# hanmekim/SceneLib2

Hardware: NVIDIA H100
Metric: EKF-SLAM frames/sec @320x240 N=100 feats (higher is better)
Workload: dtype f64 (EKF, scores) + u8/int32 (correlation sums)

## Files before the change

scenelib2_b200/csrc/update.cu:

```cuda
#include <type_traits>

#include "sl2_context.cuh"
#include "sl2_ptx.cuh"

using namespace sl2;

namespace {

constexpr int UPD_THREADS = 256;
constexpr int UPD_NB = 16;
constexpr int UPD_WS = 20;
constexpr int UPD_DS = 20;
constexpr int UPD_MS = 20;
constexpr int UPD_YS = 68;
constexpr int SOLVE_MAX_WARPS = 8;

__host__ __device__ inline int upd_keven(int kmax) { return (kmax + 1) & ~1; }
__host__ __device__ inline int upd_panw(int kmax) {
  return ((2 * upd_keven(kmax) + 15) & ~15) + 2;
}
__host__ __device__ inline size_t upd_pan_doubles(int kmax) { return (size_t)UPD_NB * upd_panw(kmax); }

__device__ __forceinline__ void dmma884(double &c0, double &c1, double a, double b) {
  asm("mma.sync.aligned.m8n8k4.row.col.f64.f64.f64.f64 {%0,%1}, {%2}, {%3}, {%0,%1};"
      : "+d"(c0), "+d"(c1)
      : "d"(a), "d"(b));
}
__device__ __forceinline__ void dmma1684(double (&c)[4], const double (&a)[2], double b) {
  asm("mma.sync.aligned.m16n8k4.row.col.f64.f64.f64.f64 {%0,%1,%2,%3}, {%4,%5}, {%6}, {%0,%1,%2,%3};"
      : "+d"(c[0]), "+d"(c[1]), "+d"(c[2]), "+d"(c[3])
      : "d"(a[0]), "d"(a[1]), "d"(b));
}
__device__ __forceinline__ void dmma1688(double (&c)[4], const double (&a)[4], const double (&b)[2]) {
  asm("mma.sync.aligned.m16n8k8.row.col.f64.f64.f64.f64 {%0,%1,%2,%3}, {%4,%5,%6,%7}, {%8,%9}, {%0,%1,%2,%3};"
      : "+d"(c[0]), "+d"(c[1]), "+d"(c[2]), "+d"(c[3])
      : "d"(a[0]), "d"(a[1]), "d"(a[2]), "d"(a[3]), "d"(b[0]), "d"(b[1]));
}
__device__ __forceinline__ void cp_async_commit() { asm volatile("cp.async.commit_group;" ::: "memory"); }
template <int N>
__device__ __forceinline__ void cp_async_wait() {
  asm volatile("cp.async.wait_group %0;" ::"n"(N) : "memory");
}
__device__ __forceinline__ void bulk_g2s(void *smem_dst, const void *gsrc, uint32_t bytes, uint32_t bar) {
  asm volatile("cp.async.bulk.shared::cluster.global.mbarrier::complete_tx::bytes [%0], [%1], %2, [%3];" ::"r"(
                   smem_u32(smem_dst)),
               "l"(gsrc), "r"(bytes), "r"(bar)
               : "memory");
}

__device__ __forceinline__ double pivot_rsqrt(double dv) {
  double y;
  asm("rsqrt.approx.ftz.f64 %0, %1;" : "=d"(y) : "d"(dv));
#pragma unroll
  for (int it = 0; it < 2; ++it) {
    const double e = fma(-(dv * y), y, 1.0);
    y = fma(0.5 * y, e, y);
  }
  return y;
}

__device__ __forceinline__ void chol8_inv(double *dg, double *Wm, int o, int lane) {
  const int j = lane & 7;
  double a[8], w[8];
#pragma unroll
  for (int i = 0; i < 8; ++i) {
    a[i] = (i <= j) ? dg[(o + i) * UPD_DS + o + j] : 0.0;
    w[i] = (i == j) ? 1.0 : 0.0;
  }
#pragma unroll
  for (int r = 0; r < 8; ++r) {
    const double dv = __shfl_sync(0xffffffffu, a[r], r);
    const double iu = pivot_rsqrt(dv);
    const double urj = a[r] * iu;
    a[r] = urj;
    w[r] *= iu;
#pragma unroll
    for (int i = r + 1; i < 8; ++i) {
      const double uri = __shfl_sync(0xffffffffu, urj, i);
      a[i] -= uri * urj;
      w[i] -= uri * w[r];
    }
  }
  __syncwarp();
  if (lane < 8) {
#pragma unroll
    for (int i = 0; i < 8; ++i) {
      if (i <= j) dg[(o + i) * UPD_DS + o + j] = a[i];
      Wm[(o + i) * UPD_WS + o + j] = w[i];
    }
  }
}

constexpr int HP_THREADS = 320;
constexpr int HP_ROWS = 16;
constexpr int HP_HRS = 18;
struct HpSmem {
  double *Hrow;
  double *Rv;
  double *nu;
  double *hprow;
  int *mfeat;
  int *wcount;
  double *park;
};
struct HpLayout {
  size_t Hrow, Rv, nu, hprow, mfeat, wcount, park, bytes;
};
__host__ __device__ inline HpLayout hp_layout(int kmax, int ld, int kd_park) {
  const size_t K = upd_keven(kmax);
  HpLayout l;
  l.Hrow = 0;
  l.Rv = l.Hrow + 2 * K * HP_HRS * sizeof(double);
  l.nu = l.Rv + 3 * K * sizeof(double);
  l.hprow = l.nu + 2 * K * sizeof(double);
  l.mfeat = l.hprow + (size_t)HP_ROWS * ld * sizeof(double);
  l.wcount = l.mfeat + K * sizeof(int);
  l.park = l.wcount + 16 * sizeof(int);
  l.bytes = l.park + (size_t)kd_park * HP_THREADS * sizeof(double);
  return l;
}
__device__ __forceinline__ HpSmem hp_carve(uint8_t *base, int kmax, int ld) {
  const HpLayout l = hp_layout(kmax, ld, 0);
  HpSmem u;
  u.Hrow = reinterpret_cast<double *>(base + l.Hrow);
  u.Rv = reinterpret_cast<double *>(base + l.Rv);
  u.nu = reinterpret_cast<double *>(base + l.nu);
  u.hprow = reinterpret_cast<double *>(base + l.hprow);
  u.mfeat = reinterpret_cast<int *>(base + l.mfeat);
  u.wcount = reinterpret_cast<int *>(base + l.wcount);
  u.park = reinterpret_cast<double *>(base + l.park);
  return u;
}

__device__ __forceinline__ int hp_tables(const Sl2Dev &d, const HpSmem &sm, int s, int rows_per_block, int row_found,
                                         int staged_m,
                                         const int *st_feat, const double *st_Hxv, const double *st_Hy,
                                         const double *st_R, const double *st_nu, const Sl2Subpix &sp,
                                         const Sl2Iter &it) {
  const int tid = threadIdx.x;
  const size_t fb = (size_t)s * d.Nmax;
  const bool iter_rows = it.h && staged_m < 0 && row_found == 1;
  const bool iter_pass = iter_rows && it.pass >= 0;
  const bool skip = iter_pass && !(it.pass == 0 ? it.max_it[s] > 0 : it.active[s] != 0);
  const bool relin = iter_rows && it.pass != 0 && it.max_it[s] > 0 && it.iters[s] > 0;
  const double *const tab_h = relin ? it.h : d.h;
  const double *const tab_dxp = relin ? it.Hxp : d.dh_dxp;
  const double *const tab_dy = relin ? it.Hy : d.dh_dy;
  int K;
  if (staged_m >= 0) {
    K = staged_m / 2;
    for (int k = tid; k < K; k += HP_THREADS) sm.mfeat[k] = st_feat[k];
  } else {
    const int nsel = d.nsel[s];
    int feat = -1;
    if (!skip && tid < d.Nmax && tid < nsel) {
      const int i = d.job_feat[fb + tid];
      if (i >= 0 && d.found[fb + i] == row_found) feat = i;
    }
    K = block_gather(feat, sm.mfeat, sm.wcount, (SL2_MAX_MEASURED + 31) / 32);
  }
  const int m = 2 * K;
  if (blockIdx.x == 0 && tid == 0) {
    d.upd_m[s] = m;
    if (staged_m < 0 && row_found == 1) {
      if (!iter_pass) d.nmeas[s] = K;
    } else if (staged_m < 0 && K > 0) {
      d.nmeas[s] += K;
    }
// ... 427 lines not shown
          chol8_inv(dg, sm.Wm, 0, lane);
          __syncwarp();
          {
            double c0 = 0.0, c1 = 0.0;
#pragma unroll
            for (int ks = 0; ks < 2; ++ks)
              dmma884(c0, c1, sm.Wm[lr * UPD_WS + 4 * ks + lc], dg[(4 * ks + lc) * UPD_DS + 8 + lr]);
            __syncwarp();
            *reinterpret_cast<double2 *>(dg + lr * UPD_DS + 8 + 2 * lc) = make_double2(c0, c1);
          }
          __syncwarp();
          {
            double2 cv = *reinterpret_cast<const double2 *>(dg + (8 + lr) * UPD_DS + 8 + 2 * lc);
#pragma unroll
            for (int ks = 0; ks < 2; ++ks) {
              const double v = dg[(4 * ks + lc) * UPD_DS + 8 + lr];
              dmma884(cv.x, cv.y, -v, v);
            }
            *reinterpret_cast<double2 *>(dg + (8 + lr) * UPD_DS + 8 + 2 * lc) = cv;
          }
          __syncwarp();
          chol8_inv(dg, sm.Wm, 8, lane);
          __syncwarp();
          {
            double t0 = 0.0, t1 = 0.0;
#pragma unroll
            for (int ks = 0; ks < 2; ++ks)
              dmma884(t0, t1, dg[(4 * ks + lc) * UPD_DS + 8 + lr], sm.Wm[(4 * ks + lc) * UPD_WS + lr]);
            *reinterpret_cast<double2 *>(dg + (8 + lr) * UPD_DS + 2 * lc) = make_double2(t0, t1);
            __syncwarp();
            double w0 = 0.0, w1 = 0.0;
#pragma unroll
            for (int ks = 0; ks < 2; ++ks)
              dmma884(w0, w1, -sm.Wm[(8 + lr) * UPD_WS + 8 + 4 * ks + lc], dg[(8 + 4 * ks + lc) * UPD_DS + lr]);
            *reinterpret_cast<double2 *>(sm.Wm + (8 + lr) * UPD_WS + 2 * lc) = make_double2(w0, w1);
          }
          __syncwarp();
          if (nbp < UPD_NB)
            for (int e = lane; e < UPD_NB * UPD_NB; e += 32) {
              const int i = e >> 4, j = e & 15;
              if (i >= nbp || j >= nbp) sm.Wm[i * UPD_WS + j] = 0.0;
            }
        }
      } else if (it == 1) {
        if (nbn == 0) continue;
        double c[2][4];
#pragma unroll
        for (int q = 0; q < 2; ++q)
#pragma unroll
          for (int mt = 0; mt < 2; ++mt) {
            const int r = mt * 8 + lr, cc = 8 * q + 2 * lc;
            c[q][2 * mt] = (r < nbn && n0 + cc < width) ? G[(size_t)(n0 + r) * ldg + n0 + cc] : 0.0;
            c[q][2 * mt + 1] = (r < nbn && n0 + cc + 1 < width) ? G[(size_t)(n0 + r) * ldg + n0 + cc + 1] : 0.0;
          }
        double v[CH_D][2];
        const size_t kstride = (size_t)4 * ldg;
        const double *gpre = G + (size_t)lc * ldg + n0 + lr;
        double *mp = mnext + lc * UPD_MS + lr;
        const bool v0 = lr < nbn, v1 = 8 + lr < nbn;
        auto loadv = [&](double *dst) {
          const double x0 = gpre[0], x1 = gpre[8];
          dst[0] = v0 ? -x0 : 0.0;
          dst[1] = v1 ? -x1 : 0.0;
          gpre += kstride;
        };
        auto step = [&](const double *vu) {
          const double a[2] = {vu[0], vu[1]};
          mp[0] = a[0];
          mp[8] = a[1];
          mp += 4 * UPD_MS;
          dmma1684(c[0], a, -a[0]);
          dmma1684(c[1], a, -a[1]);
        };
#pragma unroll
        for (int u = 0; u < CH_D - 1; ++u)
          if (u < nk) loadv(v[u]);
        int kb = 0;
        for (; kb + CH_D <= nk; kb += CH_D) {
#pragma unroll
          for (int u = 0; u < CH_D; ++u) {
            if (kb + u + CH_D - 1 < nk) loadv(v[(u + CH_D - 1) % CH_D]);
            step(v[u]);
          }
        }
#pragma unroll
        for (int q = 0; q < 2; ++q)
#pragma unroll
          for (int mt = 0; mt < 2; ++mt)
            *reinterpret_cast<double2 *>(dnext + (mt * 8 + lr) * CH_DPS + 8 * q + 2 * lc) =
                make_double2(c[q][2 * mt], c[q][2 * mt + 1]);
      } else {
        const int bt = it - 2;
        if (gb == 4) chol_batch<4, 4>(G, ldg, mcur, sm.pan, PW, i0, nbp, nk, ngroups, width, 2 + bt * 4, lr, lc);
        else if (gb == 2) chol_batch<2, 8>(G, ldg, mcur, sm.pan, PW, i0, nbp, nk, ngroups, width, 2 + bt * 2, lr, lc);
        else chol_batch<1, 8>(G, ldg, mcur, sm.pan, PW, i0, nbp, nk, ngroups, width, 2 + bt, lr, lc);
      }
    }
    __syncthreads();
    const int ncol = width - i0;
    for (int e = tid; e < UPD_NB * UPD_NB; e += UPD_THREADS) {
      const int r = e / UPD_NB, cc = e - r * UPD_NB;
      if (r < nbp && cc < nbp && i0 + cc < width)
        G[(size_t)(i0 + r) * ldg + i0 + cc] = (cc >= r) ? sm.dg[r * UPD_DS + cc] : 0.0;
      Wp[(size_t)pidx * 256 + e] = sm.Wm[r * UPD_WS + cc];
      if (r >= nbp || UPD_NB + cc >= ncol) mnext[(i0 + r) * UPD_MS + cc] = 0.0;
    }
    if (tid == 0) s_next = 1;
    {
      double aw[4][2];
#pragma unroll
      for (int mt = 0; mt < 2; ++mt)
#pragma unroll
        for (int ks = 0; ks < 4; ++ks) aw[ks][mt] = sm.Wm[(mt * 8 + lr) * UPD_WS + 4 * ks + lc];
      constexpr int FG = 4;
      for (int gb = 2 + warp; gb * 8 < ncol; gb += FG * (UPD_THREADS / 32)) {
        double c[FG][4];
#pragma unroll
        for (int f = 0; f < FG; ++f) c[f][0] = c[f][1] = c[f][2] = c[f][3] = 0.0;
#pragma unroll
        for (int ks = 0; ks < 4; ++ks) {
          double bv[FG];
#pragma unroll
          for (int f = 0; f < FG; ++f) {
            const int cb = (gb + f * (UPD_THREADS / 32)) * 8 + lr;
            bv[f] = cb < ncol ? sm.pan[(size_t)(4 * ks + lc) * PW + cb] : 0.0;
          }
#pragma unroll
          for (int f = 0; f < FG; ++f) dmma1684(c[f], aw[ks], bv[f]);
        }
#pragma unroll
        for (int f = 0; f < FG; ++f) {
          const int gq = gb + f * (UPD_THREADS / 32);
          const int cc = gq * 8 + 2 * lc;
#pragma unroll
          for (int mt = 0; mt < 2; ++mt) {
            const int r = mt * 8 + lr;
            if (r < nbp && cc < ncol) {
              double *dst = G + (size_t)(i0 + r) * ldg + i0 + cc;
              if (cc + 1 < ncol) *reinterpret_cast<double2 *>(dst) = make_double2(c[f][2 * mt], c[f][2 * mt + 1]);
              else *dst = c[f][2 * mt];
              if (gq < 4) {
                mnext[(i0 + r) * UPD_MS + cc - UPD_NB] = -c[f][2 * mt];
                if (cc + 1 < ncol) mnext[(i0 + r) * UPD_MS + cc + 1 - UPD_NB] = -c[f][2 * mt + 1];
              }
            }
          }
        }
      }
    }
    __syncthreads();
  }
}

__device__ __forceinline__ double c_to_b(const double (&c)[2][2], int ks, int lane) {
  const int lr = lane >> 2, lc = lane & 3;
  const int src = ((4 * (ks & 1) + lc) << 2) | (lr >> 1);
  const double v0 = __shfl_sync(0xffffffffu, c[ks >> 1][0], src);
  const double v1 = __shfl_sync(0xffffffffu, c[ks >> 1][1], src);
  return (lr & 1) ? v1 : v0;
}

template <int NP> struct SolveLayout {
  static constexpr int SPLIT = NP > 13 ? 6 : NP;
  static constexpr int REUSE = NP > 13 ? 4 : NP;
  __host__ __device__ static constexpr int pw(int p) { return 16 * (NP - 1 - p) + 4; }
  __host__ __device__ static constexpr int off_lin(int p0, int p) {
    int o = 0;
    for (int q = p0; q < p; ++q) o += 16 * pw(q);
    return o;
  }
  __host__ __device__ static constexpr int off(int p) { return p < SPLIT ? off_lin(0, p) : off_lin(SPLIT, p); }
  static constexpr int PAN_DOUBLES = off_lin(0, SPLIT < NP - 1 ? SPLIT : NP - 1);
  static constexpr int SMEM_DOUBLES = PAN_DOUBLES + NP * 16 * UPD_WS + NP + (NP & 1) +
                                      2 * SOLVE_MAX_WARPS * 2 * 32 * 2 +
                                      SOLVE_MAX_WARPS * 128;
  static_assert(SPLIT == NP || off_lin(SPLIT, NP - 1) <= off_lin(0, REUSE), "second generation must fit");
};

template <int NP>
__global__ void __launch_bounds__(64 * SOLVE_MAX_WARPS, 1) upd_solve_kernel(const Sl2Dev d, int stream_lo) {
  using L = SolveLayout<NP>;
  extern __shared__ __align__(16) uint8_t smem_raw[];
  pdl_prologue();
  double *pan = reinterpret_cast<double *>(smem_raw);
  double *Wm = pan + L::PAN_DOUBLES;
  const uint32_t bars = smem_u32(Wm + NP * 16 * UPD_WS);
  double2 *xbuf = reinterpret_cast<double2 *>(Wm + NP * 16 * UPD_WS + NP + (NP & 1));
  double *ybuf = reinterpret_cast<double *>(xbuf + 2 * SOLVE_MAX_WARPS * 2 * 32);
  const int s = stream_lo + blockIdx.y;
  const int m = d.upd_m[s];
  if (m == 0) return;
  const int tid = threadIdx.x, nthr = blockDim.x;
  const int ngrp = nthr >> 6;
  const int warp = tid >> 5, lane = tid & 31, lr = lane >> 2, lc = lane & 3;
  const int g = warp % ngrp, rho = warp / ngrp;
  const int n = SL2_NXV + 3 * d.nfeat[s];
  const int ncols = n + 1;
  if (blockIdx.x * ngrp * 8 >= ncols) return;
  const int ldg = d.ldg;
  double *__restrict__ G = d.G + (size_t)s * d.mmax * ldg;
  const double *__restrict__ Wp = d.Wp + (size_t)s * SL2_MAX_PANELS * 256;
  const int m8 = (m + 7) & ~7;
  const bool full = L::SPLIT == NP && m8 >= 16 * NP - 8;
  const int zend = full ? 16 * NP : m8;

  if (tid == 0) {
    for (int p = 0; p < NP; ++p) mbar_init(bars + 8 * p, 1);
    fence_barrier_init();
    fence_proxy_async();
  }
  auto zero_pads = [&](int plo, int phi) {
    for (int e = tid; e < (phi - plo) * 16; e += nthr) {
      const int p = plo + (e >> 4), r = e & 15;
      const int cfirst = 16 * p + 16;
      if (16 * p < m)
        for (int c = max(m, cfirst); c < zend; ++c) pan[L::off(p) + r * L::pw(p) + (c - cfirst)] = 0.0;
    }
  };
  zero_pads(0, L::SPLIT);
  __syncthreads();
  auto request = [&](int p) {
    if (16 * p < m) {
      const int cfirst = 16 * p + 16;
      const int nrow = min(16, m - 16 * p);
      const uint32_t ubytes = m > cfirst ? (uint32_t)(m - cfirst) * 8u : 0u;
      const uint32_t bar = bars + 8 * p;
      if (lane == 0) mbar_expect_tx(bar, (uint32_t)nrow * ubytes + 16u * 128u);
      __syncwarp();
      if (lane < 16) {
        if (lane < nrow && ubytes)
          bulk_g2s(pan + L::off(p) + lane * L::pw(p), G + (size_t)(16 * p + lane) * ldg + cfirst, ubytes, bar);
      } else {
        bulk_g2s(Wm + ((size_t)p * 16 + (lane - 16)) * UPD_WS, Wp + (size_t)p * 256 + (lane - 16) * 16, 128u, bar);
      }
    }
  };
  if (warp == 0) {
#pragma unroll 1
    for (int p = 0; p < L::SPLIT; ++p) request(p);
  }

  int xpar = 0;
  auto solve_group = [&](auto full_c, const int grp) {
    constexpr bool FULL = decltype(full_c)::value;
    const int c0 = 8 * grp;
    const bool wact = c0 < ncols;
    const int cc = c0 + 2 * lc;
    const int cval = wact ? min(2, ncols - cc) : 0;
    double *gcol = G + m + cc;
    double acc[(NP + 1) & ~1][2];
    {
      const int ccn = cc + 8 * (int)(gridDim.x * ngrp);
      if (L::SPLIT >= NP && ccn < ncols) {
#pragma unroll
        for (int t = 0; t < NP; ++t) {
          const int row = 8 * (2 * t + rho) + lr;
          if (row < m) asm volatile("prefetch.global.L2 [%0];" ::"l"(G + m + ccn + (size_t)row * ldg));
        }
      }
    }
#pragma unroll
    for (int t = 0; t < ((NP + 1) & ~1); ++t) {
      const int row = 8 * (2 * t + rho) + lr;
      acc[t][0] = acc[t][1] = 0.0;
      if (row < m) {
        if (cval >= 2) {
          const double2 v = *reinterpret_cast<const double2 *>(gcol + (size_t)row * ldg);
          acc[t][0] = v.x;
          acc[t][1] = v.y;
        } else if (cval == 1) {
          acc[t][0] = gcol[(size_t)row * ldg];
        }
      }
    }

#pragma unroll
    for (int p = 0; p < NP; ++p) {
      if (FULL || 16 * p < m) {
        if (L::SPLIT < NP && p == L::REUSE) {
          __syncthreads();
          zero_pads(L::SPLIT, NP);
          __syncthreads();
          if (warp == 0) {
            fence_proxy_async();
#pragma unroll 1
            for (int q = L::SPLIT; q < NP; ++q) request(q);
          }
        }
        if (!wact) continue;
        xpar ^= 1;
        double2 *xb = xbuf + ((size_t)(xpar * ngrp + g) * 2) * 32;
        xb[rho * 32 + lane] = make_double2(acc[p][0], acc[p][1]);
        asm volatile("bar.sync %0, 64;" ::"r"(1 + g) : "memory");
        const double2 other = xb[(rho ^ 1) * 32 + lane];
        const double cp2[2][2] = {{rho ? other.x : acc[p][0], rho ? other.y : acc[p][1]},
                                  {rho ? acc[p][0] : other.x, rho ? acc[p][1] : other.y}};
        mbar_wait(bars + 8 * p, 0);
        const double *pb = pan + L::off(p);
        const int PW = L::pw(p);
        const double *wb = Wm + (size_t)p * 16 * UPD_WS;
        double cb[4];
#pragma unroll
        for (int ks = 0; ks < 4; ++ks) cb[ks] = c_to_b(cp2, ks, lane);
        double d0 = 0.0, d1 = 0.0;
#pragma unroll
        for (int ks = 0; ks < 4; ++ks) dmma884(d0, d1, wb[(8 * rho + lr) * UPD_WS + 4 * ks + lc], cb[ks]);
        {
          const int row = 16 * p + 8 * rho + lr;
          if (row < m) {
            if (cval >= 2) *reinterpret_cast<double2 *>(gcol + (size_t)row * ldg) = make_double2(d0, d1);
            else if (cval == 1) gcol[(size_t)row * ldg] = d0;
          }
        }
        if (p + 1 < NP) {
          double *yg = ybuf + (size_t)g * 128;
          *reinterpret_cast<double2 *>(yg + (8 * rho + lr) * 8 + 2 * lc) = make_double2(d0, d1);
          asm volatile("bar.sync %0, 64;" ::"r"(1 + g) : "memory");
          double yb[4];
#pragma unroll
          for (int ks = 0; ks < 4; ++ks) yb[ks] = -yg[(4 * ks + lc) * 8 + lr];
          const double *pbr = pb + 8 * rho + lr;
#pragma unroll
          for (int ks = 0; ks < 4; ++ks) {
#pragma unroll
            for (int t = (p + 1) & ~1; t < NP; t += 2) {
              const bool has[2] = {t > p && (FULL || 8 * (2 * t + rho) < m),
                                   t + 1 < NP && (FULL || 8 * (2 * t + 2 + rho) < m)};
              if (has[0] || has[1]) {
                double a[2];
#pragma unroll
                for (int h = 0; h < 2; ++h) a[h] = has[h] ? pbr[(4 * ks + lc) * PW + 16 * (t + h - p - 1)] : 0.0;
                double c[4] = {acc[t][0], acc[t][1], acc[t + 1][0], acc[t + 1][1]};
                dmma1684(c, a, yb[ks]);
                acc[t][0] = c[0];
                acc[t][1] = c[1];
                acc[t + 1][0] = c[2];
                acc[t + 1][1] = c[3];
              }
            }
          }
        }
      }
    }
  };
  for (int grp = blockIdx.x * ngrp + g; L::SPLIT < NP ? grp == (int)(blockIdx.x * ngrp + g) : 8 * grp < ncols;
       grp += gridDim.x * ngrp) {
    if (L::SPLIT == NP && full) solve_group(std::true_type{}, grp);
    else solve_group(std::false_type{}, grp);
  }
}

constexpr int SYRK_THREADS = 128;
template <int KC, int ST>
__global__ void __launch_bounds__(SYRK_THREADS, 3) upd_syrk_kernel(const Sl2Dev d, int stream_lo) {
  constexpr int STAGE = 2 * KC * UPD_YS;
  constexpr int NW = SYRK_THREADS / 32;
  extern __shared__ __align__(16) uint8_t smem_raw[];
  double *stage_buf = reinterpret_cast<double *>(smem_raw);
  pdl_prologue();
  const int s = stream_lo + blockIdx.y;
  const int m = d.upd_m[s];
  if (m == 0) return;
  const int n = SL2_NXV + 3 * d.nfeat[s];
  int tb = 0;
  const int t = blockIdx.x;
  while ((tb + 1) * (tb + 2) / 2 <= t) ++tb;
  const int ta = t - tb * (tb + 1) / 2;
  if (tb * 64 >= n + 1) return;
  const int tid = threadIdx.x, warp = tid >> 5, lane = tid & 31, lr = lane >> 2, lc = lane & 3;
  const int wa = (warp & 1) * 32, wb = (warp >> 1) * 32;
  const int ld = d.ld, ldg = d.ldg;
  double *__restrict__ P = d.P + (size_t)s * ld * ld;
  double *__restrict__ x = d.x + (size_t)s * ld;
  const double *__restrict__ G = d.G + (size_t)s * d.mmax * ldg;
  const bool diag = ta == tb;
  const int bi0 = wa >> 3, bj0 = wb >> 3;
  unsigned cmask = 0xFFFFu, mmask = 0xFFFFu;
  if (diag) {
    cmask = mmask = 0u;
#pragma unroll
    for (int bi = 0; bi < 4; ++bi)
#pragma unroll
      for (int bj = 0; bj < 4; ++bj) {
        if (bi0 + bi <= bj0 + bj) cmask |= 1u << (4 * bi + bj);
        if (bi0 + bi < bj0 + bj) mmask |= 1u << (4 * bi + bj);
      }
  }
  const bool skip = cmask == 0u;
  if (!skip) {
#pragma unroll
    for (int i = 0; i < 4; ++i) {
      const int a = ta * 64 + wa + i * 8, bq = tb * 64 + wb + lane;
      if (a < n && bq < n) asm volatile("prefetch.global.L2 [%0];" ::"l"(P + a + (size_t)ld * bq));
    }
  }
  const int kr = m, lim = m + n + 1;
  const int nchunk = (kr + KC - 1) / KC;
  const int cA = m + ta * 64 + 2 * lane, cB = m + tb * 64 + 2 * lane;
  const int bytesA = cA + 1 < lim ? 16 : (cA < lim ? 8 : 0);
  const int bytesB = cB + 1 < lim ? 16 : (cB < lim ? 8 : 0);
  const double *srcA = G + (bytesA ? cA : 0);
  const double *srcB = G + (bytesB ? cB : 0);
  const double *pa = srcA + (size_t)warp * ldg, *pb = srcB + (size_t)warp * ldg;
  const uint32_t sdst = smem_u32(stage_buf + 2 * lane + warp * UPD_YS);
  const size_t rstep = (size_t)NW * ldg;
  auto stage = [&](int chunk) {
    const uint32_t dd = sdst + (uint32_t)(chunk % ST) * (STAGE * 8);
    if ((chunk + 1) * KC <= kr) {
#pragma unroll
      for (int j = 0; j < KC / NW; ++j) {
        asm volatile("cp.async.cg.shared.global [%0], [%1], 16, %2;" ::"r"(dd + j * NW * UPD_YS * 8),
                     "l"(pa + j * rstep), "r"(bytesA)
                     : "memory");
        if (!diag)
          asm volatile("cp.async.cg.shared.global [%0], [%1], 16, %2;" ::"r"(dd + (KC + j * NW) * UPD_YS * 8),
                       "l"(pb + j * rstep), "r"(bytesB)
                       : "memory");
      }
    } else {
#pragma unroll
      for (int j = 0; j < KC / NW; ++j) {
        const bool kv = chunk * KC + warp + NW * j < kr;
        asm volatile("cp.async.cg.shared.global [%0], [%1], 16, %2;" ::"r"(dd + j * NW * UPD_YS * 8),
                     "l"(kv ? pa + j * rstep : srcA), "r"(kv ? bytesA : 0)
                     : "memory");
        if (!diag)
          asm volatile("cp.async.cg.shared.global [%0], [%1], 16, %2;" ::"r"(dd + (KC + j * NW) * UPD_YS * 8),
                       "l"(kv ? pb + j * rstep : srcB), "r"(kv ? bytesB : 0)
                       : "memory");
      }
    }
    pa += (size_t)KC * ldg;
    pb += (size_t)KC * ldg;
  };
  double acc[2][4][4];
#pragma unroll
  for (int i = 0; i < 2; ++i)
#pragma unroll
    for (int j = 0; j < 4; ++j)
#pragma unroll
      for (int e = 0; e < 4; ++e) acc[i][j][e] = 0.0;
#pragma unroll
  for (int c = 0; c < ST - 1; ++c) {
    if (c < nchunk) stage(c);
    cp_async_commit();
  }
  for (int ch = 0; ch < nchunk; ++ch) {
    cp_async_wait<ST - 2>();
    __syncthreads();
    if (ch + ST - 1 < nchunk) stage(ch + ST - 1);
    cp_async_commit();
    if (!skip) {
      const double *Ya = stage_buf + (size_t)(ch % ST) * STAGE;
      const double *Yb = diag ? Ya : Ya + KC * UPD_YS;
      const int krem = kr - ch * KC;
      auto chunk = [&](auto diag_c) {
        constexpr bool DIAG = decltype(diag_c)::value;
        auto kstep = [&](int kk) {
          double a[2][4], b[4][2];
#pragma unroll
          for (int i = 0; i < 2; ++i)
#pragma unroll
            for (int e = 0; e < 4; ++e)
              a[i][e] = Ya[(kk + lc + 4 * (e >> 1)) * UPD_YS + wa + 16 * i + 8 * (e & 1) + lr];
#pragma unroll
          for (int j = 0; j < 4; ++j)
#pragma unroll
            for (int e = 0; e < 2; ++e) b[j][e] = Yb[(kk + lc + 4 * e) * UPD_YS + wb + j * 8 + lr];
#pragma unroll
          for (int i = 0; i < 2; ++i)
#pragma unroll
            for (int j = 0; j < 4; ++j)
              if (!DIAG || 2 * i <= j) dmma1688(acc[i][j], a[i], b[j]);
        };
        if (krem >= KC) {
#pragma unroll
          for (int kk = 0; kk < KC; kk += 8) kstep(kk);
        } else {
#pragma unroll 1
          for (int kk = 0; kk < krem; kk += 8) kstep(kk);
        }
      };
      if (cmask == 0xFFFFu) chunk(std::false_type{});
      else chunk(std::true_type{});
    }
  }
  if (skip) return;
#pragma unroll
  for (int bi = 0; bi < 4; ++bi) {
    const int i = bi >> 1, h = bi & 1;
    const int a = ta * 64 + wa + bi * 8 + lr;
    double pold[4][2];
#pragma unroll
    for (int j = 0; j < 4; ++j)
#pragma unroll
      for (int e = 0; e < 2; ++e) {
        const int bq = tb * 64 + wb + j * 8 + 2 * lc + e;
        pold[j][e] = (((cmask >> (4 * bi + j)) & 1u) && a < n && bq < n) ? P[a + (size_t)ld * bq] : 0.0;
      }
#pragma unroll
    for (int j = 0; j < 4; ++j) {
      if (!((cmask >> (4 * bi + j)) & 1u)) continue;
      const int bq = tb * 64 + wb + j * 8 + 2 * lc;
      const double c0 = acc[i][j][2 * h], c1 = acc[i][j][2 * h + 1];
      const double v0 = pold[j][0] - c0, v1 = pold[j][1] - c1;
      if (a < n && bq < n) {
        P[a + (size_t)ld * bq] = v0;
        if (bq + 1 < n) P[a + (size_t)ld * (bq + 1)] = v1;
        if ((mmask >> (4 * bi + j)) & 1u) {
          double *dst = P + bq + (size_t)ld * a;
          if (bq + 1 < n) *reinterpret_cast<double2 *>(dst) = make_double2(v0, v1);
          else *dst = v0;
        }
      }
      if (a < n) {
        if (bq == n) x[a] += c0;
        if (bq + 1 == n) x[a] += c1;
      }
    }
  }
}

__global__ void __launch_bounds__(UPD_THREADS) upd_finish_kernel(const Sl2Dev d, int stream_lo, int staged,
                                                                  int only_normalise, int rescued) {
  pdl_prologue();
  const int s = stream_lo + blockIdx.x;
  const int tid = threadIdx.x;
  const int nf = d.nfeat[s];
  const int n = SL2_NXV + 3 * nf;
  const int ld = d.ld;
  double *__restrict__ P = d.P + (size_t)s * ld * ld;
  const double *__restrict__ x = d.x + (size_t)s * ld;
  const size_t fb = (size_t)s * d.Nmax;
  const int m = only_normalise ? 0 : d.upd_m[s];
  if (rescued && m == 0) return;
  __shared__ int s_cull;
  if (m > 0 || only_normalise) {
    __shared__ double J4[16];
    if (tid == 0) {
      const rd q[4] = {rd(x[3]), rd(x[4]), rd(x[5]), rd(x[6])};
      const rd qq = q[0] * q[0] + q[1] * q[1] + q[2] * q[2] + q[3] * q[3];
      for (int i = 0; i < 4; ++i)
        for (int j = 0; j < 4; ++j)
          J4[i * 4 + j] = (i == j) ? ((rd(1.0) - q[i] * q[i] / (qq * qq)) / qq).v
                                   : ((-q[i]) * q[j] / (qq * qq * qq)).v;
    }
    __syncthreads();
    for (int j = tid; j < n; j += UPD_THREADS) {
      double v[4], o[4];
      for (int k = 0; k < 4; ++k) v[k] = P[(3 + k) + (size_t)ld * j];
      for (int i = 0; i < 4; ++i) {
        rd a(0.0);
        for (int k = 0; k < 4; ++k) a = a + rd(J4[i * 4 + k]) * rd(v[k]);
        o[i] = a.v;
      }
      for (int k = 0; k < 4; ++k) P[(3 + k) + (size_t)ld * j] = o[k];
    }
    __syncthreads();
    for (int i = tid; i < n; i += UPD_THREADS) {
      if (i < SL2_NXV) {
        double v[4], o[4];
        for (int k = 0; k < 4; ++k) v[k] = P[i + (size_t)ld * (3 + k)];
        for (int c = 0; c < 4; ++c) {
          rd a(0.0);
          for (int k = 0; k < 4; ++k) a = a + rd(v[k]) * rd(J4[c * 4 + k]);
          o[c] = a.v;
        }
        for (int k = 0; k < 4; ++k) P[i + (size_t)ld * (3 + k)] = o[k];
      } else {
        for (int k = 0; k < 4; ++k) P[i + (size_t)ld * (3 + k)] = P[(3 + k) + (size_t)ld * i];
      }
    }
    __syncthreads();
  }
  {
    const int i = tid % 13, j = (tid / 13) % 13;
    const double a = P[i + (size_t)ld * j], b = P[j + (size_t)ld * i];
    const double v = (rd(a) * rd(0.5) + rd(b) * rd(0.5)).v;
    __syncthreads();
    if (tid < 169) P[i + (size_t)ld * j] = v;
    __syncthreads();
  }
  if (!staged && !only_normalise) {
    if (tid == 0) s_cull = 0;
    __syncthreads();
    for (int i = tid; i < nf; i += UPD_THREADS) {
      int att = d.attempted[fb + i], suc = d.successful[fb + i];
      if (rescued) {
        if (d.found[fb + i] == SL2_FOUND_RESCUED) {
          suc += 1;
          d.successful[fb + i] = suc;
          d.found[fb + i] = 1;
        }
      } else if (d.sel_rank[fb + i] >= 0) {
        att += 1;
        if (d.found[fb + i] == 1) suc += 1;
        d.attempted[fb + i] = att;
        d.successful[fb + i] = suc;
      }
      if (att >= d.min_attempts && (double)suc / (double)att < d.match_fraction) atomicAdd(&s_cull, 1);
    }
    __syncthreads();
    if (tid == 0) d.ncull[s] = s_cull;
  }
}

struct SolveKernel {
  void (*kern)(Sl2Dev, int);
  int np;
  size_t smem;
};
template <int NP>
SolveKernel solve_kernel_np() {
  return {upd_solve_kernel<NP>, NP, SolveLayout<NP>::SMEM_DOUBLES * sizeof(double)};
}
inline SolveKernel solve_kernel(int kmax) {
  const int p = (2 * upd_keven(kmax) + 15) / 16;
  return p <= 4 ? solve_kernel_np<4>()
                : (p <= 7 ? solve_kernel_np<7>()
                          : (p <= 10 ? solve_kernel_np<10>() : (p <= 13 ? solve_kernel_np<13>() : solve_kernel_np<16>())));
}
inline void solve_shape(int Nmax, int &nslab, int &warps) {
  const int ngroups = (SL2_NXV + 3 * Nmax + 1 + 7) / 8;
  nslab = (ngroups + SOLVE_MAX_WARPS - 1) / SOLVE_MAX_WARPS;
  warps = (ngroups + nslab - 1) / nslab;
}
constexpr size_t SYRK_SMEM = (size_t)2 * 2 * 32 * UPD_YS * sizeof(double);

size_t sl2_update_smem_bytes(const Sl2Dev &d) {
  return chol_smem_doubles(d.kmax) * sizeof(double);
}

}

cudaError_t sl2_configure_update(const Sl2Dev &d) {
  const SolveKernel solve = solve_kernel(d.kmax);
  const struct {
    const void *kern;
    size_t smem;
  } opt_in[] = {
      {(const void *)upd_hp_kernel<7>, hp_layout(d.kmax, d.ld, 0).bytes},
      {(const void *)upd_hp_kernel<13>, hp_layout(d.kmax, d.ld, 0).bytes},
      {(const void *)upd_hp2_kernel<7>, hp_layout(d.kmax, d.ld, 7).bytes},
      {(const void *)upd_hp2_kernel<13>, hp_layout(d.kmax, d.ld, 13).bytes},
      {(const void *)upd_chol_kernel, sl2_update_smem_bytes(d)},
      {(const void *)solve.kern, solve.smem},
      {(const void *)upd_syrk_kernel<32, 2>, SYRK_SMEM},
  };
  for (const auto &k : opt_in) {
    const cudaError_t e = cudaFuncSetAttribute(k.kern, cudaFuncAttributeMaxDynamicSharedMemorySize, (int)k.smem);
    if (e != cudaSuccess) return e;
  }
  return cudaSuccess;
}

namespace {

cudaError_t launch_hp(const Sl2Dev &d, int stream_lo, int stream_cnt, int row_found, int staged_m, const int *st_feat,
                      const double *st_Hxv, const double *st_Hy, const double *st_R, const double *st_nu,
                      const Sl2Subpix &sp, const Sl2Iter &it, Sl2Queue q) {
  const int hp_all = (2 * upd_keven(d.kmax) + HP_ROWS - 1) / HP_ROWS;
  const int hp_blocks = stream_cnt >= 2 * d.nsm ? 1 : hp_all;
  const dim3 grid(hp_blocks, stream_cnt);
  const bool piped = hp_blocks == 1 && SL2_NXV + 3 * d.Nmax <= HP_THREADS;
  const int kd = staged_m >= 0 ? 13 : 7;
  auto *k13 = piped ? upd_hp2_kernel<13> : upd_hp_kernel<13>;
  auto *k7 = piped ? upd_hp2_kernel<7> : upd_hp_kernel<7>;
  const size_t smem = hp_layout(d.kmax, d.ld, piped ? kd : 0).bytes;
  return sl2_launch_kernel(kd == 13 ? k13 : k7, grid, dim3(HP_THREADS), smem, q, sl2_use_pdl(stream_cnt), d, stream_lo,
                           row_found, staged_m, st_feat, st_Hxv, st_Hy, st_R, st_nu, sp, it);
}

cudaError_t launch_chol(const Sl2Dev &d, int stream_lo, int stream_cnt, Sl2Queue q) {
  return sl2_launch_kernel(upd_chol_kernel, dim3(stream_cnt), dim3(UPD_THREADS), sl2_update_smem_bytes(d), q,
                           sl2_use_pdl(stream_cnt), d, stream_lo);
}

cudaError_t launch_update(const Sl2Dev &d, int stream_lo, int stream_cnt, int row_found, int staged_m,
                          const int *st_feat, const double *st_Hxv, const double *st_Hy, const double *st_R,
                          const double *st_nu, int only_normalise, const Sl2Subpix &sp, const Sl2Iter &it, Sl2Queue q,
                          cudaEvent_t *ev6) {
  if (stream_cnt <= 0) return cudaSuccess;
  cudaError_t e;
  auto mark = [&](int i) { return ev6 ? cudaEventRecord(ev6[i], q.stream) : cudaSuccess; };
  if ((e = mark(0)) != cudaSuccess) return e;
  const bool pdl = sl2_use_pdl(stream_cnt);
  if (!only_normalise) {
    e = launch_hp(d, stream_lo, stream_cnt, row_found, staged_m, st_feat, st_Hxv, st_Hy, st_R, st_nu, sp, it, q);
    if (e != cudaSuccess) return e;
  }
  if ((e = mark(1)) != cudaSuccess) return e;
  if (!only_normalise) {
    e = launch_chol(d, stream_lo, stream_cnt, q);
    if (e != cudaSuccess) return e;
  }
  if ((e = mark(2)) != cudaSuccess) return e;
  if (!only_normalise) {
    int nslab, warps;
    solve_shape(d.Nmax, nslab, warps);
    const SolveKernel solve = solve_kernel(d.kmax);
    const bool walk = solve.np <= 13 && stream_cnt >= d.nsm;
    if (walk) warps = SOLVE_MAX_WARPS;
    e = sl2_launch_kernel(solve.kern, dim3(walk ? 1 : nslab, stream_cnt), dim3(64 * warps), solve.smem, q, pdl, d,
                          stream_lo);
    if (e != cudaSuccess) return e;
  }
  if ((e = mark(3)) != cudaSuccess) return e;
  if (!only_normalise) {
    const int nt = (SL2_NXV + 3 * d.Nmax + 1 + 63) / 64;
    e = sl2_launch_kernel(upd_syrk_kernel<32, 2>, dim3(nt * (nt + 1) / 2, stream_cnt), dim3(SYRK_THREADS), SYRK_SMEM,
                          q, pdl, d, stream_lo);
    if (e != cudaSuccess) return e;
  }
  if ((e = mark(4)) != cudaSuccess) return e;
  e = sl2_launch_kernel(upd_finish_kernel, dim3(stream_cnt), dim3(UPD_THREADS), 0, q, pdl, d, stream_lo,
                        (int)(staged_m >= 0), only_normalise, (int)(row_found == SL2_FOUND_RESCUED));
  if (e != cudaSuccess) return e;
  if ((e = mark(5)) != cudaSuccess) return e;
  return cudaGetLastError();
}

}

cudaError_t sl2_launch_update(const Sl2Dev &d, int stream_lo, int stream_cnt, int staged_m,
                              const int *st_feat, const double *st_Hxv, const double *st_Hy,
                              const double *st_R, const double *st_nu, int only_normalise,
                              const Sl2Subpix &sp, Sl2Queue q, cudaEvent_t *ev6, const Sl2Iter &it) {
  return launch_update(d, stream_lo, stream_cnt, 1, staged_m, st_feat, st_Hxv, st_Hy, st_R, st_nu, only_normalise, sp,
                       it, q, ev6);
}

cudaError_t sl2_launch_iterate_factor(const Sl2Dev &d, int stream_lo, int stream_cnt, const Sl2Subpix &sp,
                                      const Sl2Iter &it, Sl2Queue q) {
  if (stream_cnt <= 0) return cudaSuccess;
  cudaError_t e = launch_hp(d, stream_lo, stream_cnt, 1, -1, nullptr, nullptr, nullptr, nullptr, nullptr, sp, it, q);
  if (e != cudaSuccess) return e;
  return launch_chol(d, stream_lo, stream_cnt, q);
}

cudaError_t sl2_launch_update_rescued(const Sl2Dev &d, int stream_lo, int stream_cnt, int *m2, const Sl2Subpix &sp,
                                      Sl2Queue q) {
  Sl2Dev d2 = d;
  d2.upd_m = m2;
  return launch_update(d2, stream_lo, stream_cnt, SL2_FOUND_RESCUED, -1, nullptr, nullptr, nullptr, nullptr, nullptr, 0,
                       sp, Sl2Iter{}, q, nullptr);
}

extern "C" {

int sl2_ekf_update(sl2_ctx *c, int32_t s, int32_t m, const int32_t *feat_index, const double *H_xv,
                   const double *H_y, const double *R, const double *nu) {
  if (bad_stream(c, s) || m < 0 || (m & 1) || m > c->d.mmax)
    return fail(c, SL2_ERR_ARG, "sl2_ekf_update: bad m");
  if (m == 0) return SL2_OK;
  if (!feat_index || !H_xv || !H_y || !R || !nu) return fail(c, SL2_ERR_ARG, "sl2_ekf_update: null argument");
  const int K = m / 2;
  int nf = 0;
  int rc = device_nfeat(c, s, &nf);
  if (rc) return rc;
  for (int k = 0; k < K; ++k) {
    if (feat_index[k] < 0 || feat_index[k] >= nf) return fail(c, SL2_ERR_ARG, "sl2_ekf_update: bad feature index");
    if (R[k * 4 + 1] != R[k * 4 + 2]) return fail(c, SL2_ERR_ARG, "sl2_ekf_update: R block is not symmetric");
  }
  const size_t k = K;
  Stage hx{STAGE_IN, 8 * 26 * k, H_xv}, hy{STAGE_IN, 8 * 6 * k, H_y}, r{STAGE_IN, 8 * 4 * k, R},
      v{STAGE_IN, 8 * 2 * k, nu}, fe{STAGE_IN, 4 * k, feat_index};
  return staged_call(c, {&hx, &hy, &r, &v, &fe}, [] {}, [&] {
    CU_TRY(c, sl2_launch_update(c->d, s, 1, m, fe.dev<int>(), hx.dev<double>(), hy.dev<double>(), r.dev<double>(),
                                v.dev<double>(), 0, Sl2Subpix{}, queue(c)));
    return SL2_OK;
  });
}

int sl2_ekf_update_measured(sl2_ctx *c, int32_t s) {
  if (bad_stream(c, s)) return fail(c, SL2_ERR_ARG, "bad stream");
  const int rc0 = iterate_streams(c, s, 1, queue(c));
  if (rc0) return rc0;
  CU_TRY(c, sl2_launch_update(c->d, s, 1, -1, nullptr, nullptr, nullptr, nullptr, nullptr, 0, subpixel_args(c, s, 1),
                              queue(c), nullptr, iterate_args(c, s, 1)));
  if (rescue_on(c, s, 1)) {
    const int rc = rescue_streams(c, s, 1, queue(c));
    if (rc) return rc;
  }
  CU_TRY(c, cudaStreamSynchronize(c->stream));
  return SL2_OK;
}

int sl2_normalise_state(sl2_ctx *c, int32_t s) {
  if (bad_stream(c, s)) return fail(c, SL2_ERR_ARG, "bad stream");
  CU_TRY(c, sl2_launch_update(c->d, s, 1, -1, nullptr, nullptr, nullptr, nullptr, nullptr, 1, Sl2Subpix{}, queue(c)));
  CU_TRY(c, cudaStreamSynchronize(c->stream));
  return SL2_OK;
}

}
```

Measured before the change: 233,700.

## Restructure triangular solve into 4-warp quads over 16-column groups

Measured after the change: 233,700, median of 6. Within noise of the previous version (-0.0%).

```diff
diff --git a/scenelib2_b200/csrc/update.cu b/scenelib2_b200/csrc/update.cu
--- a/scenelib2_b200/csrc/update.cu
+++ b/scenelib2_b200/csrc/update.cu
@@ -13,7 +13,7 @@
 constexpr int UPD_DS = 20;
 constexpr int UPD_MS = 20;
 constexpr int UPD_YS = 68;
-constexpr int SOLVE_MAX_WARPS = 8;
+constexpr int SOLVE_MAX_QUADS = 4;
 
 __host__ __device__ inline int upd_keven(int kmax) { return (kmax + 1) & ~1; }
 __host__ __device__ inline int upd_panw(int kmax) {
@@ -747,14 +747,7 @@
   }
 }
 
-__device__ __forceinline__ double c_to_b(const double (&c)[2][2], int ks, int lane) {
-  const int lr = lane >> 2, lc = lane & 3;
-  const int src = ((4 * (ks & 1) + lc) << 2) | (lr >> 1);
-  const double v0 = __shfl_sync(0xffffffffu, c[ks >> 1][0], src);
-  const double v1 = __shfl_sync(0xffffffffu, c[ks >> 1][1], src);
-  return (lr & 1) ? v1 : v0;
-}
-
+constexpr int SOLVE_XS = 20;
 template <int NP> struct SolveLayout {
   static constexpr int SPLIT = NP > 13 ? 6 : NP;
   static constexpr int REUSE = NP > 13 ? 4 : NP;
@@ -767,31 +760,33 @@
   __host__ __device__ static constexpr int off(int p) { return p < SPLIT ? off_lin(0, p) : off_lin(SPLIT, p); }
   static constexpr int PAN_DOUBLES = off_lin(0, SPLIT < NP - 1 ? SPLIT : NP - 1);
   static constexpr int SMEM_DOUBLES = PAN_DOUBLES + NP * 16 * UPD_WS + NP + (NP & 1) +
-                                      2 * SOLVE_MAX_WARPS * 2 * 32 * 2 +
-                                      SOLVE_MAX_WARPS * 128;
+                                      2 * SOLVE_MAX_QUADS * 16 * SOLVE_XS +
+                                      SOLVE_MAX_QUADS * 16 * SOLVE_XS;
   static_assert(SPLIT == NP || off_lin(SPLIT, NP - 1) <= off_lin(0, REUSE), "second generation must fit");
+  static_assert(SMEM_DOUBLES * 8 <= 227 * 1024, "one CTA per SM");
 };
 
 template <int NP>
-__global__ void __launch_bounds__(64 * SOLVE_MAX_WARPS, 1) upd_solve_kernel(const Sl2Dev d, int stream_lo) {
+__global__ void __launch_bounds__(128 * SOLVE_MAX_QUADS, 1) upd_solve_kernel(const Sl2Dev d, int stream_lo) {
   using L = SolveLayout<NP>;
+  constexpr int NT = (NP + 1) / 2;
   extern __shared__ __align__(16) uint8_t smem_raw[];
   pdl_prologue();
   double *pan = reinterpret_cast<double *>(smem_raw);
   double *Wm = pan + L::PAN_DOUBLES;
   const uint32_t bars = smem_u32(Wm + NP * 16 * UPD_WS);
-  double2 *xbuf = reinterpret_cast<double2 *>(Wm + NP * 16 * UPD_WS + NP + (NP & 1));
-  double *ybuf = reinterpret_cast<double *>(xbuf + 2 * SOLVE_MAX_WARPS * 2 * 32);
+  double *xbuf = Wm + NP * 16 * UPD_WS + NP + (NP & 1);
+  double *ybuf = xbuf + 2 * SOLVE_MAX_QUADS * 16 * SOLVE_XS;
   const int s = stream_lo + blockIdx.y;
   const int m = d.upd_m[s];
   if (m == 0) return;
   const int tid = threadIdx.x, nthr = blockDim.x;
-  const int ngrp = nthr >> 6;
+  const int ngq = nthr >> 7;
   const int warp = tid >> 5, lane = tid & 31, lr = lane >> 2, lc = lane & 3;
-  const int g = warp % ngrp, rho = warp / ngrp;
+  const int gq = warp >> 2, q = warp & 3;
   const int n = SL2_NXV + 3 * d.nfeat[s];
   const int ncols = n + 1;
-  if (blockIdx.x * ngrp * 8 >= ncols) return;
+  if (blockIdx.x * ngq * 16 >= ncols) return;
   const int ldg = d.ldg;
   double *__restrict__ G = d.G + (size_t)s * d.mmax * ldg;
   const double *__restrict__ Wp = d.Wp + (size_t)s * SL2_MAX_PANELS * 256;
@@ -838,37 +833,46 @@
   int xpar = 0;
   auto solve_group = [&](auto full_c, const int grp) {
     constexpr bool FULL = decltype(full_c)::value;
-    const int c0 = 8 * grp;
+    const int c0 = 16 * grp;
     const bool wact = c0 < ncols;
-    const int cc = c0 + 2 * lc;
-    const int cval = wact ? min(2, ncols - cc) : 0;
-    double *gcol = G + m + cc;
-    double acc[(NP + 1) & ~1][2];
+    int cval[2];
+#pragma unroll
+    for (int h = 0; h < 2; ++h) cval[h] = wact ? min(2, ncols - (c0 + 8 * h + 2 * lc)) : 0;
+    double *gcol = G + m + c0 + 2 * lc;
+    double acc[NT][2][2];
     {
-      const int ccn = cc + 8 * (int)(gridDim.x * ngrp);
-      if (L::SPLIT >= NP && ccn < ncols) {
-#pragma unroll
-        for (int t = 0; t < NP; ++t) {
-          const int row = 8 * (2 * t + rho) + lr;
-          if (row < m) asm volatile("prefetch.global.L2 [%0];" ::"l"(G + m + ccn + (size_t)row * ldg));
-        }
-      }
-    }
-#pragma unroll
-    for (int t = 0; t < ((NP + 1) & ~1); ++t) {
-      const int row = 8 * (2 * t + rho) + lr;
-      acc[t][0] = acc[t][1] = 0.0;
-      if (row < m) {
-        if (cval >= 2) {
-          const double2 v = *reinterpret_cast<const double2 *>(gcol + (size_t)row * ldg);
-          acc[t][0] = v.x;
-          acc[t][1] = v.y;
-        } else if (cval == 1) {
-          acc[t][0] = gcol[(size_t)row * ldg];
-        }
-      }
-    }
-
+      const int ccn = c0 + 2 * lc + 16 * (int)(gridDim.x * ngq);
+      if (L::SPLIT >= NP) {
+#pragma unroll
+        for (int t = 0; t < NT; ++t) {
+          const int row = 8 * (4 * t + q) + lr;
+#pragma unroll
+          for (int h = 0; h < 2; ++h)
+            if (row < m && ccn + 8 * h < ncols)
+              asm volatile("prefetch.global.L2 [%0];" ::"l"(G + m + ccn + 8 * h + (size_t)row * ldg));
+        }
+      }
+    }
+#pragma unroll
+    for (int t = 0; t < NT; ++t) {
+      const int row = 8 * (4 * t + q) + lr;
+#pragma unroll
+      for (int h = 0; h < 2; ++h) {
+        acc[t][h][0] = acc[t][h][1] = 0.0;
+        if (row < m) {
+          const double *src = gcol + 8 * h + (size_t)row * ldg;
+          if (cval[h] >= 2) {
+            const double2 v = *reinterpret_cast<const double2 *>(src);
+            acc[t][h][0] = v.x;
+            acc[t][h][1] = v.y;
+          } else if (cval[h] == 1) {
+            acc[t][h][0] = *src;
+          }
+        }
+      }
+    }
+
+    const int r2 = q & 1, hq = q >> 1;
 #pragma unroll
     for (int p = 0; p < NP; ++p) {
       if (FULL || 16 * p < m) {
@@ -879,58 +883,73 @@
           if (warp == 0) {
             fence_proxy_async();
 #pragma unroll 1
-            for (int q = L::SPLIT; q < NP; ++q) request(q);
+            for (int q2 = L::SPLIT; q2 < NP; ++q2) request(q2);
           }
         }
         if (!wact) continue;
         xpar ^= 1;
-        double2 *xb = xbuf + ((size_t)(xpar * ngrp + g) * 2) * 32;
-        xb[rho * 32 + lane] = make_double2(acc[p][0], acc[p][1]);
-        asm volatile("bar.sync %0, 64;" ::"r"(1 + g) : "memory");
-        const double2 other = xb[(rho ^ 1) * 32 + lane];
-        const double cp2[2][2] = {{rho ? other.x : acc[p][0], rho ? other.y : acc[p][1]},
-                                  {rho ? acc[p][0] : other.x, rho ? acc[p][1] : other.y}};
+        double *xb = xbuf + (size_t)(xpar * SOLVE_MAX_QUADS + gq) * 16 * SOLVE_XS;
+        if ((q >> 1) == (p & 1)) {
+#pragma unroll
+          for (int h = 0; h < 2; ++h)
+            *reinterpret_cast<double2 *>(xb + (8 * r2 + lr) * SOLVE_XS + 8 * h + 2 * lc) =
+                make_double2(acc[p >> 1][h][0], acc[p >> 1][h][1]);
+        }
+        asm volatile("bar.sync %0, 128;" ::"r"(1 + gq) : "memory");
         mbar_wait(bars + 8 * p, 0);
         const double *pb = pan + L::off(p);
         const int PW = L::pw(p);
         const double *wb = Wm + (size_t)p * 16 * UPD_WS;
-        double cb[4];
-#pragma unroll
-        for (int ks = 0; ks < 4; ++ks) cb[ks] = c_to_b(cp2, ks, lane);
         double d0 = 0.0, d1 = 0.0;
 #pragma unroll
-        for (int ks = 0; ks < 4; ++ks) dmma884(d0, d1, wb[(8 * rho + lr) * UPD_WS + 4 * ks + lc], cb[ks]);
+        for (int ks = 0; ks < 4; ++ks)
+          dmma884(d0, d1, wb[(8 * r2 + lr) * UPD_WS + 4 * ks + lc], xb[(4 * ks + lc) * SOLVE_XS + 8 * hq + lr]);
         {
-          const int row = 16 * p + 8 * rho + lr;
+          const int row = 16 * p + 8 * r2 + lr;
           if (row < m) {
-            if (cval >= 2) *reinterpret_cast<double2 *>(gcol + (size_t)row * ldg) = make_double2(d0, d1);
-            else if (cval == 1) gcol[(size_t)row * ldg] = d0;
+            double *dst = gcol + 8 * hq + (size_t)row * ldg;
+            const int cv = hq ? cval[1] : cval[0];
+            if (cv >= 2) *reinterpret_cast<double2 *>(dst) = make_double2(d0, d1);
+            else if (cv == 1) *dst = d0;
           }
         }
         if (p + 1 < NP) {
-          double *yg = ybuf + (size_t)g * 128;
-          *reinterpret_cast<double2 *>(yg + (8 * rho + lr) * 8 + 2 * lc) = make_double2(d0, d1);
-          asm volatile("bar.sync %0, 64;" ::"r"(1 + g) : "memory");
-          double yb[4];
-#pragma unroll
-          for (int ks = 0; ks < 4; ++ks) yb[ks] = -yg[(4 * ks + lc) * 8 + lr];
-          const double *pbr = pb + 8 * rho + lr;
+          double *yg = ybuf + (size_t)gq * 16 * SOLVE_XS;
+          *reinterpret_cast<double2 *>(yg + (8 * r2 + lr) * SOLVE_XS + 8 * hq + 2 * lc) = make_double2(d0, d1);
+          asm volatile("bar.sync %0, 128;" ::"r"(1 + gq) : "memory");
+          double yb[2][4];
+#pragma unroll
+          for (int h = 0; h < 2; ++h)
+#pragma unroll
+            for (int ks = 0; ks < 4; ++ks) yb[h][ks] = -yg[(4 * ks + lc) * SOLVE_XS + 8 * h + lr];
+          const double *pbr = pb + 8 * q + lr - 16 * (p + 1);
 #pragma unroll
           for (int ks = 0; ks < 4; ++ks) {
 #pragma unroll
-            for (int t = (p + 1) & ~1; t < NP; t += 2) {
-              const bool has[2] = {t > p && (FULL || 8 * (2 * t + rho) < m),
-                                   t + 1 < NP && (FULL || 8 * (2 * t + 2 + rho) < m)};
+            for (int u = 0; 2 * u < NT; ++u) {
+              bool has[2];
+#pragma unroll
+              for (int hh = 0; hh < 2; ++hh) {
+                const int t = 2 * u + hh, j = 4 * t + q;
+                has[hh] = t < NT && 4 * t + 3 >= 2 * p + 2 && (4 * t >= 2 * p + 2 || j >= 2 * p + 2) &&
+                          (4 * t + 3 < 2 * NP || j < 2 * NP) && (FULL || 8 * j < m);
+              }
               if (has[0] || has[1]) {
                 double a[2];
 #pragma unroll
-                for (int h = 0; h < 2; ++h) a[h] = has[h] ? pbr[(4 * ks + lc) * PW + 16 * (t + h - p - 1)] : 0.0;
-                double c[4] = {acc[t][0], acc[t][1], acc[t + 1][0], acc[t + 1][1]};
-                dmma1684(c, a, yb[ks]);
-                acc[t][0] = c[0];
-                acc[t][1] = c[1];
-                acc[t + 1][0] = c[2];
-                acc[t + 1][1] = c[3];
+                for (int hh = 0; hh < 2; ++hh) a[hh] = has[hh] ? pbr[(4 * ks + lc) * PW + 32 * (2 * u + hh)] : 0.0;
+#pragma unroll
+                for (int h = 0; h < 2; ++h) {
+                  double c[4] = {acc[2 * u][h][0], acc[2 * u][h][1], 2 * u + 1 < NT ? acc[2 * u + 1][h][0] : 0.0,
+                                 2 * u + 1 < NT ? acc[2 * u + 1][h][1] : 0.0};
+                  dmma1684(c, a, yb[h][ks]);
+                  acc[2 * u][h][0] = c[0];
+                  acc[2 * u][h][1] = c[1];
+                  if (2 * u + 1 < NT) {
+                    acc[2 * u + 1][h][0] = c[2];
+                    acc[2 * u + 1][h][1] = c[3];
+                  }
+                }
               }
             }
           }
@@ -938,8 +957,8 @@
       }
     }
   };
-  for (int grp = blockIdx.x * ngrp + g; L::SPLIT < NP ? grp == (int)(blockIdx.x * ngrp + g) : 8 * grp < ncols;
-       grp += gridDim.x * ngrp) {
+  for (int grp = blockIdx.x * ngq + gq; L::SPLIT < NP ? grp == (int)(blockIdx.x * ngq + gq) : 16 * grp < ncols;
+       grp += gridDim.x * ngq) {
     if (L::SPLIT == NP && full) solve_group(std::true_type{}, grp);
     else solve_group(std::false_type{}, grp);
   }
@@ -1215,10 +1234,10 @@
                 : (p <= 7 ? solve_kernel_np<7>()
                           : (p <= 10 ? solve_kernel_np<10>() : (p <= 13 ? solve_kernel_np<13>() : solve_kernel_np<16>())));
 }
-inline void solve_shape(int Nmax, int &nslab, int &warps) {
-  const int ngroups = (SL2_NXV + 3 * Nmax + 1 + 7) / 8;
-  nslab = (ngroups + SOLVE_MAX_WARPS - 1) / SOLVE_MAX_WARPS;
-  warps = (ngroups + nslab - 1) / nslab;
+inline void solve_shape(int Nmax, int &nslab, int &quads) {
+  const int ngroups = (SL2_NXV + 3 * Nmax + 1 + 15) / 16;
+  nslab = (ngroups + SOLVE_MAX_QUADS - 1) / SOLVE_MAX_QUADS;
+  quads = (ngroups + nslab - 1) / nslab;
 }
 constexpr size_t SYRK_SMEM = (size_t)2 * 2 * 32 * UPD_YS * sizeof(double);
 
@@ -1291,12 +1310,12 @@
   }
   if ((e = mark(2)) != cudaSuccess) return e;
   if (!only_normalise) {
-    int nslab, warps;
-    solve_shape(d.Nmax, nslab, warps);
+    int nslab, quads;
+    solve_shape(d.Nmax, nslab, quads);
     const SolveKernel solve = solve_kernel(d.kmax);
     const bool walk = solve.np <= 13 && stream_cnt >= d.nsm;
-    if (walk) warps = SOLVE_MAX_WARPS;
-    e = sl2_launch_kernel(solve.kern, dim3(walk ? 1 : nslab, stream_cnt), dim3(64 * warps), solve.smem, q, pdl, d,
+    if (walk) quads = SOLVE_MAX_QUADS;
+    e = sl2_launch_kernel(solve.kern, dim3(walk ? 1 : nslab, stream_cnt), dim3(128 * quads), solve.smem, q, pdl, d,
                           stream_lo);
     if (e != cudaSuccess) return e;
   }
```
